# Sachin-A/TraceWeaver

Measured on AMD Instinct MI355X. Metric: spans/sec reconstructed + assignment accuracy vs ground truth, higher is better.
Workload: dtype int64 timestamps, f64 scores; 1 GPU; media_microservices shape (6 services, E in {1,1,1,1,2,4}), 100000 requests/service x 16 replicas per GPU, concurrency 1.6, two-pass reconstruction, device mixture refit; spans_per_gpu=25600000, spans_total=25600000, parallelism=units sharded, 1 rank(s), backend none

## Files before the change

### traceweaver_amd/csrc/tw_device.h

```cpp
#pragma once
#include <hip/hip_runtime.h>
#include <stdint.h>

#include "traceweaver_amd.h"

namespace tw {

constexpr int kMaxEp = TW_MAX_EP;
constexpr int kTopK = TW_TOPK;
constexpr int kMaxComp = TW_MAX_COMP;
constexpr int kMaxWin = TW_MAX_WINDOW;
constexpr int kCandWords = TW_CAND_WORDS;
constexpr int kEnumStretches = 8;
constexpr int kTile = 128;
constexpr int kCoop = 256;
constexpr int32_t kNoOwner = 0x7f7f7f7f;

struct UnitDev {
    int64_t in_off;
    int64_t ie_off;
    int64_t ep_off[kMaxEp + 1];
    int32_t n_in;
    int32_t E;
    int32_t nblk;
// ... 60 lines not shown
    int32_t* tkr_n;
    int32_t *tk_idx, *tkr_idx;
    double *tk_score, *tkr_score;
    int32_t* c_lo;
    int32_t* c_hi;
    uint64_t* c_bits;
    uint64_t* gone;
    uint8_t* gone_valid;
    int64_t* leaves_r;
    unsigned long long* frontier_big;
    int32_t* frontier_big_busy;
    int32_t frontier_big_slots;
    int32_t* frontier_busy;
    unsigned long long* frontier;
    int32_t* round_changed;
    int32_t* parent;
    int32_t* owner;
    double* gaps;
    const int64_t* gs_off;
    int64_t* unit_stats;
    int32_t* heavy_count;
    int32_t* heavy_next;
    int32_t *heavy_unit, *heavy_win;
    int32_t *tiny_unit, *tiny_win;
    int32_t *rheavy_unit, *rheavy_win, *rtiny_unit, *rtiny_win;
    int32_t *hard_unit, *hard_win;
    int32_t* heavy_in_count;
    int32_t* heavy_in_next;
    int32_t heavy_in_off[kMaxEp + 2];
    int32_t* enum_snap;
    int32_t* enum_stretch_next;
    int32_t *heavy_in_unit, *heavy_in_idx;
    int32_t* heavy_big_count;
    int32_t *heavy_big_unit, *heavy_big_idx;
    int32_t heavy_big_off[kMaxEp + 2];
    int32_t* heavy_big_part;
    int32_t* heavy_big_slot;
    int32_t part_off[kMaxEp + 2];
    int32_t split_twins;
    int32_t* part_used;
    int32_t defer_min_e;
    int32_t defer_cap;
    unsigned long long* defer_list;
    int32_t* defer_used;
    int32_t* defer_count;
    int32_t *part_lo, *part_hi;
    int32_t* part_lvl;
    int32_t* any_wide;
    int32_t* redo_count;
    int32_t* defer_refused;
    int32_t lean_min_e;
    int32_t tile_max_deep;
    int32_t lean_grid;
    double* pair_pool;
    int32_t* pair_busy;
    int32_t* fb_count;
    int32_t* fb_total;
    int32_t *fb_unit, *fb_idx, *fb_part, *fb_slot;
    int32_t* split_count;
    int32_t *split_unit, *split_idx, *split_slot, *split_parts;
    int32_t* part_n;
    int64_t* part_leaves;
    double* part_score;
    int32_t* part_idx;
    unsigned long long* part_bits;
    int32_t* part_logn;
    double* part_log_sc;
    unsigned long long* part_log_ix;
    int32_t* err;
    unsigned long long* prof;
};

__device__ __forceinline__ int32_t hi_word(double x) { return (int32_t)(__double_as_longlong(x) >> 32); }
__device__ __forceinline__ uint32_t lo_word(double x) { return (uint32_t)__double_as_longlong(x); }
__device__ __forceinline__ double with_hi(double x, int32_t hi) {
    return __longlong_as_double((long long)(((uint64_t)(uint32_t)hi << 32) | (uint64_t)lo_word(x)));
}
__device__ __forceinline__ double dnan() { return __longlong_as_double(0x7ff8000000000000LL); }
__device__ __forceinline__ double dinf() { return __longlong_as_double(0x7ff0000000000000LL); }

__device__ inline double tw_log(double x) {
    const double ln2_hi = 6.93147180369123816490e-01, ln2_lo = 1.90821492927058770002e-10,
                 two54 = 1.80143985094819840000e+16, Lg1 = 6.666666666666735130e-01,
                 Lg2 = 3.999999999940941908e-01, Lg3 = 2.857142874366239149e-01,
                 Lg4 = 2.222219843214978396e-01, Lg5 = 1.818357216161805012e-01,
                 Lg6 = 1.531383769920937332e-01, Lg7 = 1.479819860511658591e-01;
    int32_t k = 0, hx = hi_word(x);
    if (hx < 0x00100000) {
        if (((hx & 0x7fffffff) | lo_word(x)) == 0) return -dinf();
        if (hx < 0) return dnan();
        k -= 54;
        x *= two54;
        hx = hi_word(x);
    }
    if (hx >= 0x7ff00000) return x + x;
    k += (hx >> 20) - 1023;
    hx &= 0x000fffff;
    int32_t i = (hx + 0x95f64) & 0x100000;
    x = with_hi(x, hx | (i ^ 0x3ff00000));
    k += (i >> 20);
    double f = x - 1.0, dk = (double)k;
    if ((0x000fffff & (2 + hx)) < 3) {
        if (f == 0.0) return k == 0 ? 0.0 : dk * ln2_hi + dk * ln2_lo;
        double R = f * f * (0.5 - 0.33333333333333333 * f);
        return k == 0 ? f - R : dk * ln2_hi - ((R - dk * ln2_lo) - f);
    }
// ... 169 lines not shown
```

### traceweaver_amd/csrc/tw_engine.hip

```cpp
#include <algorithm>
#include <chrono>
#include <cmath>
#include <cstdio>
#include <cstdlib>
#include <cstring>
#include <functional>
#include <string>
#include <type_traits>
#include <vector>

#include <hip/hip_runtime.h>
#include <rocprim/rocprim.hpp>

#include "traceweaver_amd.h"
#include "tw_kernels.h"
#include "tw_fit.h"
#include "tw_eval.h"
#include "tw_skip.h"
#include "tw_load.h"
#include "tw_baselines.h"
#include "tw_stitch.h"
#include "tw_attr.h"
#include "tw_conf.h"
#include "tw_dist.h"
// ... 25 lines not shown
    uint32_t next() {
        if (idx >= 624) {
            for (int i = 0; i < 624; i++) {
                const uint32_t y = (mt[i] & 0x80000000u) | (mt[(i + 1) % 624] & 0x7fffffffu);
                mt[i] = mt[(i + 397) % 624] ^ (y >> 1) ^ ((y & 1u) ? 0x9908b0dfu : 0u);
            }
            idx = 0;
        }
        uint32_t y = mt[idx++];
        y ^= y >> 11;
        y ^= (y << 7) & 0x9d2c5680u;
        y ^= (y << 15) & 0xefc60000u;
        y ^= y >> 18;
        return y;
    }
    double random_sample() {
        const uint32_t a = next() >> 5, b = next() >> 6;
        return ((double)a * 67108864.0 + (double)b) / 9007199254740992.0;
    }
};

}

struct tw_engine {
    int device = 0;
    hipStream_t stream = nullptr;
    hipStream_t cls_stream[kMaxEp + 1] = {};
    hipEvent_t cls_ev[kMaxEp + 2] = {};
    hipStream_t sel_stream[3] = {};
    hipStream_t sel_stream2[3] = {};
    int64_t select_fork_min = 0;
    hipEvent_t prep_ev = nullptr;
    hipEvent_t post_fork[kMaxEp + 1] = {}, post_join[kMaxEp + 1][3] = {}, post_done[kMaxEp + 1] = {};
    hipEvent_t tile_ev[kMaxEp + 1] = {};
    hipStream_t cls_stream2[kMaxEp + 1] = {};
    hipEvent_t stretch_ev[kMaxEp + 1][kEnumStretches] = {}, stretch_done[kMaxEp + 1] = {};
    int enum_stretches = 1, stretch_min_tiles = 2048;
    int heavy_grid = 4096, select_grid = 0;
    int debug_lists = 0;
    int32_t first_lists[3][kMaxEp + 1] = {};
    hipEvent_t gate_ev = nullptr;
    int tile_gate = 0;
    int stage_min_tiles = 1024;
    int32_t *rank_in = nullptr, *rank_out = nullptr;
    bool class_params = false;
    int prio_min_e = 0, prio_high = 0;
    bool prio_any = false;
    int pipeline = 1;
    std::string err;
    int state = ST_EMPTY;
    int tile = kTile;
    int tile_threads = 2;
    int tile_single = 1;
    int block_params = 1;
    int tile_single_threads = 1;
    int coop = kCoop;
    std::vector<UnitDev> units;
    std::vector<TileDev> tiles;
    std::vector<int64_t> gs_off_h;
    std::vector<void*> allocs;
    void* arena = nullptr;
    size_t arena_cap = 0;
    bool arena_open = false;
    std::vector<std::pair<std::function<void(void*)>, size_t>> arena_req;
    Dev P{};
    int64_t n_ie = 0, n_gp = 0, n_slots = 0, n_gaps = 0;
    PairVI* agg_pair = nullptr;
    int32_t *agg_i32 = nullptr, *agg_i32b = nullptr;
    uint32_t *seg_in = nullptr, *seg_out = nullptr;
    int n_seg_out = 0;
    void* sort_tmp = nullptr;
    size_t sort_tmp_bytes = 0;
    double* mix_p_dev = nullptr;
    int32_t* mix_n_dev = nullptr;
    double* mix_c_dev = nullptr;
    double* gaps_sorted = nullptr;
    double* fit_models = nullptr;
    double* fit_uval = nullptr;
    int32_t *fit_ustart = nullptr, *fit_row_n = nullptr, *fit_row_uniq = nullptr;
    double* fit_centres = nullptr;
    double *fit_tape = nullptr, *fit_tape100 = nullptr;
    int64_t* fit_tape_off = nullptr;
    int64_t fit_tape_cap = 0;
    bool fit_runs_pending = false;
    bool fit_prepared = false;
    int tile_sub_max = 8;
    int32_t hard_pass1[kMaxEp + 1] = {};
    int8_t wide_pass1[kMaxEp + 1] = {};
    int32_t split_pass1[kMaxEp + 1] = {};
    int lean_pool = 512;
    bool pass1_done = false;
    std::vector<int32_t> fit_max_n;
    bool fit_max_n_valid = false;
    Mt19937 fit_rng;
    uint32_t fit_seed = 0;
    int32_t* slot_unit = nullptr;
    int32_t* tile_ids = nullptr;
    int32_t* ctr = nullptr;
    int64_t ctr_round_ints = 0, ctr_pass_ints = 0;
    int32_t tile_cls_off[kMaxEp + 2] = {};
    BlockRef* blk_tab = nullptr;
    int32_t blk_cls_off[kMaxEp + 2] = {};
    uint32_t *seg_gap = nullptr, *seg_gap_end = nullptr, *seg_gap_dst = nullptr;
    unsigned long long *comp_a = nullptr, *comp_b = nullptr;
    int64_t comp_cap = 0, n_gap_scored = 0;
    int32_t *truth = nullptr, *in_trace = nullptr;
// ... 745 lines not shown
    const unsigned grid_in = (unsigned)std::min<int64_t>((n_in + 255) / 256, 8192), grid_out = (unsigned)std::min<int64_t>((n_out + 255) / 256, 8192);
    const unsigned block = flat_threads(e);
    int64_t* d_is = const_cast<int64_t*>(P.in_start); int64_t* d_ie = const_cast<int64_t*>(P.in_end);
    int64_t* d_os = const_cast<int64_t*>(P.out_start); int64_t* d_oe = const_cast<int64_t*>(P.out_end);
    for (int side = 0; side < 2; side++) {
        const int64_t n = side == 0 ? n_in : n_out;
        const int64_t* vs = (const int64_t*)(side == 0 ? L.x : L.y); const int64_t* ve = (const int64_t*)(side == 0 ? L.xe : L.ye);
        const int32_t* rank = side == 0 ? L.rank_in : L.rank_out; const int32_t* row = side == 0 ? L.row_in : L.row_out;
        const int nrows = side == 0 ? P.n_units : e->n_seg_out;
        unsigned bs = 0, be = 0;
        rc = differing_bits(e, vs, n, &bs); if (rc != TW_OK) return rc;
        rc = differing_bits(e, ve, n, &be); if (rc != TW_OK) return rc;
        hipLaunchKernelGGL(k_load_iota, dim3(side == 0 ? grid_in : grid_out), dim3(block), 0, e->stream, perm, n);
        rc = load_sort_pass(e, rank, n, 32u, ka, kb, &perm, &perm_alt); if (rc != TW_OK) return rc;
        rc = load_sort_pass(e, ve, n, be, ka, kb, &perm, &perm_alt); if (rc != TW_OK) return rc;
        rc = load_sort_pass(e, vs, n, bs, ka, kb, &perm, &perm_alt); if (rc != TW_OK) return rc;
        rc = load_sort_pass(e, row, n, std::max(1u, bit_length((unsigned long long)std::max(nrows - 1, 1))), ka, kb, &perm, &perm_alt); if (rc != TW_OK) return rc;
        hipLaunchKernelGGL(k_load_place, dim3(side == 0 ? grid_in : grid_out), dim3(block), 0, e->stream, (const uint32_t*)perm, n, vs, ve,
                           side == 0 ? d_is : d_os, side == 0 ? d_ie : d_oe, side == 0 ? pos_in : pos_out);
        hipLaunchKernelGGL(k_load_local, dim3(side == 0 ? grid_in : grid_out), dim3(block), 0, e->stream, perm, row, (const uint32_t*)(side == 0 ? e->seg_in : e->seg_out), n);
        HIPCHK(hipGetLastError());
        int32_t* host = side == 0 ? in_perm : out_perm;
        if (host != nullptr) HIPCHK(hipMemcpyAsync(host, perm, sizeof(uint32_t) * n, hipMemcpyDeviceToHost, e->stream));
        HIPCHK(hipStreamSynchronize(e->stream));
    }
    hipLaunchKernelGGL(k_load_retruth, dim3(P.n_tiles), dim3(e->tile), 0, e->stream, L, (const int32_t*)pos_in, (const int32_t*)pos_out, e->truth,
                       has_trace ? e->in_trace : nullptr);
    HIPCHK(hipGetLastError());
    for (int u = 0; u < P.n_units; u++) {
        UnitDev& U = e->units[(size_t)u];
        U.tscale = std::ldexp(1.0, -kmax_h[(size_t)u]);
        U.float_time = 1;
        if (unit_time_scale != nullptr) unit_time_scale[u] = U.tscale;
    }
    HIPCHK(hipMemcpyAsync(const_cast<UnitDev*>(P.units), e->units.data(), sizeof(UnitDev) * e->units.size(), hipMemcpyHostToDevice, e->stream));
    HIPCHK(hipStreamSynchronize(e->stream));
    e->state = ST_LOADED; e->pass1_done = false;
    drop_batch_order(e);
    for (int E = 0; E <= kMaxEp; E++) { e->wide_pass1[E] = -1; e->hard_pass1[E] = -1; e->split_pass1[E] = -1; }
    return TW_OK;
}

extern "C" {

int tw_create(int device_id, tw_engine** out) {
    if (out == nullptr) return TW_ERR_ARG;
    *out = nullptr;
    tw_engine* e = new tw_engine();
    e->device = device_id;
    e->tile = std::min(std::max(env_int("TW_TILE", kTile), 1), kTile);
    e->tile_threads = std::min(std::max(env_int("TW_TILE_THREADS", 2), 1), 4);
    e->tile_single = env_int("TW_TILE_SINGLE", 1);
    e->block_params = env_int("TW_BLOCK_PARAMS", 1);
    e->tile_single_threads = std::min(std::max(env_int("TW_TILE_SINGLE_THREADS", 1), 1), 4);
    e->coop = std::min(std::max(env_int("TW_COOP_THREADS", kCoop), 1), kCoop);
    if (env_int("TW_SET_HW_QUEUES", 0) != 0) setenv("GPU_MAX_HW_QUEUES", "12", 0);
    hipError_t s = hipSetDevice(device_id);
    if (s == hipSuccess) s = hipStreamCreate(&e->stream);
    for (int i = 0; i < EV_COUNT && s == hipSuccess; i++) s = hipEventCreate(&e->ev[i]);
    for (int i = 0; i < SE_COUNT && s == hipSuccess; i++) s = hipEventCreate(&e->stage_ev[i]);
    const int prio_min_e = env_int("TW_PRIO_MIN_E", 0);
    int prio_least = 0, prio_greatest = 0;
    if (s == hipSuccess) s = hipDeviceGetStreamPriorityRange(&prio_least, &prio_greatest);
    e->prio_min_e = prio_min_e; e->prio_high = prio_greatest; e->prio_any = prio_greatest != prio_least;
    for (int i = 0; i <= kMaxEp + 1 && s == hipSuccess; i++) s = hipEventCreateWithFlags(&e->cls_ev[i], hipEventDisableTiming);
    if (s == hipSuccess) s = hipEventCreateWithFlags(&e->prep_ev, hipEventDisableTiming);
    for (int i = 0; i <= kMaxEp && s == hipSuccess; i++) {
        s = hipEventCreateWithFlags(&e->post_fork[i], hipEventDisableTiming);
        if (s == hipSuccess) s = hipEventCreateWithFlags(&e->tile_ev[i], hipEventDisableTiming);
        if (s == hipSuccess) s = hipEventCreateWithFlags(&e->post_done[i], hipEventDisableTiming);
        if (s == hipSuccess) s = hipEventCreateWithFlags(&e->stretch_done[i], hipEventDisableTiming);
        for (int j = 0; j < kEnumStretches && s == hipSuccess; j++) s = hipEventCreateWithFlags(&e->stretch_ev[i][j], hipEventDisableTiming);
        for (int j = 0; j < 3 && s == hipSuccess; j++) s = hipEventCreateWithFlags(&e->post_join[i][j], hipEventDisableTiming);
    }
    e->pipeline = env_int("TW_CLASS_PIPELINE", 1);
    e->sig_hash_bits = std::min(std::max(env_int("TW_SIG_HASH_BITS", 64), 1), 64);
    e->tile_gate = env_int("TW_TILE_GATE", 0);
    e->enum_stretches = std::min(std::max(env_int("TW_ENUM_STRETCHES", 1), 1), kEnumStretches);
    e->heavy_grid = std::max(env_int("TW_HEAVY_GRID", 4096), 64);
    e->select_grid = std::max(env_int("TW_SELECT_GRID", 0), 0);
    e->debug_lists = env_int("TW_DEBUG_LISTS", 0);
    e->select_fork_min = (int64_t)env_int("TW_SELECT_FORK_MIN", 0);
    e->stretch_min_tiles = std::max(env_int("TW_STRETCH_MIN_TILES", 2048), 1);
    e->stage_min_tiles = env_int("TW_STAGE_MIN_TILES", 1024);
    e->tile_sub_max = std::max(env_int("TW_TILE_SUB", 8), 1);
    e->lean_pool = std::min(std::max(env_int("TW_LEAN_POOL", 512), 1), 4096);
    if (s != hipSuccess) {
        fprintf(stderr, "tw_create: %s\n", hipGetErrorString(s));
        delete e;
        return TW_ERR_DEVICE;
    }
    *out = e;
    return TW_OK;
}

void tw_destroy(tw_engine* e) {
    if (e == nullptr) return;
    (void)hipSetDevice(e->device);
    free_all(e);
    order_unstage(e);
    if (e->arena != nullptr) (void)hipFree(e->arena);
    for (int i = 0; i < EV_COUNT; i++)
        if (e->ev[i]) (void)hipEventDestroy(e->ev[i]);
    for (int i = 0; i <= kMaxEp + 1; i++)
        if (e->cls_ev[i]) (void)hipEventDestroy(e->cls_ev[i]);
    for (int i = 1; i <= kMaxEp; i++)
// ... 149 lines not shown
        for (int cls = 1; cls <= kMaxEp; cls++) if (e->tile_cls_off[cls + 1] > e->tile_cls_off[cls]) deepest = cls;
        for (int cls = 1; cls < deepest; cls++) want |= e->select_fork_min > 0 && heavy_off_h[cls + 1] - heavy_off_h[cls] >= e->select_fork_min;
        for (int j = 0; j < 3 && want; j++)
            if (e->sel_stream2[j] == nullptr) HIPCHK(hipStreamCreate(&e->sel_stream2[j]));
    }
    const int64_t n_in_total = b->unit_in_off[b->n_units], n_out_total = b->ep_off[epi];
    if (n_in_total >= (1ll << 31) || n_out_total >= (1ll << 31)) return fail(e, TW_ERR_ARG, "batch exceeds 2^31 spans");
    if (gaps >= (1ll << 31)) return fail(e, TW_ERR_ARG, "batch too large: sum of nslot*n_in must stay below 2^31");
    std::vector<int32_t> slot_unit_h;
    std::vector<uint8_t> slot_scored_h;
    std::vector<uint32_t> seg_gap_h, seg_gap_end_h;
    for (int u = 0; u < b->n_units; u++) {
        const UnitDev& U = e->units[(size_t)u];
        const int E = U.E;
        for (int q = 0; q < U.nslot; q++) {
            bool scored;
            if (q < E) scored = U.npred[q] == 0;
            else if (q < E + E * E) {
                const int p = (q - E) / E, en = (q - E) % E;
                scored = false;
                for (int j = 0; j < U.npred[en]; j++) scored |= (U.pred_list[en][j] == p && U.pred_prim[en][j]);
            } else scored = true;
            slot_unit_h.push_back(u);
            slot_scored_h.push_back(scored ? 1 : 0);
            if (scored) {
                seg_gap_h.push_back((uint32_t)(e->gs_off_h[(size_t)u] + (int64_t)q * U.n_in));
                seg_gap_end_h.push_back((uint32_t)(e->gs_off_h[(size_t)u] + (int64_t)(q + 1) * U.n_in));
            }
        }
    }
    e->n_gap_rows = (int64_t)seg_gap_h.size();
    std::vector<uint32_t> seg_gap_dst_h(seg_gap_h.size());
    e->n_gap_scored = 0;
    for (size_t r = 0; r < seg_gap_h.size(); r++) { seg_gap_dst_h[r] = (uint32_t)e->n_gap_scored; e->n_gap_scored += seg_gap_end_h[r] - seg_gap_h[r]; }
    seg_in[(size_t)b->n_units] = (uint32_t)n_in_total;
    seg_out.push_back((uint32_t)n_out_total);
    e->n_seg_out = (int)seg_out.size() - 1;
    e->n_ie = ie; e->n_gp = gp; e->n_slots = slots; e->n_gaps = gaps;

    Dev& P = e->P;
    P = Dev{};
    P.n_units = b->n_units;
    P.n_tiles = (int32_t)e->tiles.size();
    P.tile_spans = e->tile;
    P.n_in_total = n_in_total;
    P.n_out_total = n_out_total;
    P.batch_size = b->batch_size;
    P.batch_mis = b->batch_size_mis;
    P.split_twins = env_int("TW_SPLIT_TWINS", 2);
    P.defer_min_e = env_int("TW_DEFER_MIN_E", 5);
    P.lean_min_e = env_int("TW_LEAN_MIN_E", 5);
    P.lean_grid = std::max(env_int("TW_LEAN_GRID", TW_LEAN_GRID), 1);
    P.tile_max_deep = std::min(std::max(env_int("TW_TILE_MAX_DEEP", kTileMax), 0), kTileMax);
    int rc;
    e->arena_req.clear();
    e->arena_open = true;
    UnitDev* d_units; TileDev* d_tiles; int64_t *d_is, *d_ie, *d_os, *d_oe, *d_gs;
    DEV_ALLOC(d_units, P.n_units); DEV_ALLOC(d_tiles, P.n_tiles);
    DEV_ALLOC(d_is, n_in_total); DEV_ALLOC(d_ie, n_in_total); DEV_ALLOC(d_os, n_out_total); DEV_ALLOC(d_oe, n_out_total);
    DEV_ALLOC(d_gs, P.n_units);
    DEV_ALLOC(P.in_end_sorted, n_in_total); DEV_ALLOC(P.out_end_sorted, n_out_total);
    DEV_ALLOC(P.gparam, gp * 4);
    DEV_ALLOC(e->mix_n_dev, slots); DEV_ALLOC(e->mix_p_dev, slots * kMaxComp * 3); DEV_ALLOC(e->mix_c_dev, slots * kMaxComp * 4);
    DEV_ALLOC(P.pm_val, n_in_total); DEV_ALLOC(P.pm_idx, n_in_total); DEV_ALLOC(P.pc, n_in_total + 1); DEV_ALLOC(P.seg, n_in_total);
    DEV_ALLOC(P.win_end, n_in_total); DEV_ALLOC(P.wid, n_in_total); DEV_ALLOC(P.w_last, n_in_total);
    DEV_ALLOC(P.unit_nwin, P.n_units); DEV_ALLOC(P.w_dirty, n_in_total); DEV_ALLOC(P.w_conf, n_in_total);
    DEV_ALLOC(P.tk_n, n_in_total); DEV_ALLOC(P.leaves, n_in_total); DEV_ALLOC(P.leaves0, n_in_total); DEV_ALLOC(P.chosen, n_in_total); DEV_ALLOC(P.rep, n_in_total);
    DEV_ALLOC(P.tkr_n, n_in_total);
    DEV_ALLOC(P.tk_idx, ie * kTopK); DEV_ALLOC(P.tkr_idx, ie * kTopK);
    DEV_ALLOC(P.tk_score, n_in_total * kTopK); DEV_ALLOC(P.tkr_score, n_in_total * kTopK);
    DEV_ALLOC(P.c_lo, ie); DEV_ALLOC(P.c_hi, ie); DEV_ALLOC(P.c_bits, ie * kCandWords); DEV_ALLOC(P.parent, ie);
    DEV_ALLOC(P.gone, ie * kCandWords); DEV_ALLOC(P.gone_valid, n_in_total); DEV_ALLOC(P.leaves_r, n_in_total);
    DEV_ALLOC(P.frontier, (int64_t)kFrontierSlots * 2 * kFrontierCap); 
    P.frontier_big_slots = (int32_t)std::min<int64_t>(std::max<int64_t>(n_in_total / 16384, kFrontierBigSlots), std::max(kFrontierBigSlots, 512));
    DEV_ALLOC(P.frontier_big, (int64_t)P.frontier_big_slots * 2 * kFrontierBigCap);
    DEV_ALLOC(P.pair_pool, (int64_t)kPairSlots * kPairSpill);
    DEV_ALLOC(P.owner, n_out_total);
    DEV_ALLOC(P.gaps, gaps);
    DEV_ALLOC(e->tile_ids, (int64_t)tile_ids_h.size());
    DEV_ALLOC(e->blk_tab, (int64_t)blk_tab_h.size());
    DEV_ALLOC(P.heavy_in_unit, n_in_total); DEV_ALLOC(P.heavy_in_idx, n_in_total);
    {
        int64_t big_total = 0, slots = 0, want = 0;
        for (int cls = 0; cls <= kMaxEp; cls++) want += 2 * part_extra(cls, heavy_off_h[cls + 1] - heavy_off_h[cls]);
        static const int64_t slots_max = (int64_t)std::max(env_int("TW_PART_SLOTS_MAX", 16 << 20), 1024);
        for (int cls = 0; cls <= kMaxEp; cls++) {
            const int64_t n_cls = heavy_off_h[cls + 1] - heavy_off_h[cls];
            int64_t extra = part_extra(cls, n_cls);
            if (want > slots_max && extra > 64) extra = std::max<int64_t>((int64_t)((double)extra * (double)slots_max / (double)want), std::min<int64_t>(n_cls / 8 + 64, extra));
            P.heavy_big_off[cls] = (int32_t)big_total; P.part_off[cls] = (int32_t)slots;
            big_total += n_cls + extra; slots += 2 * extra;
        }
        P.heavy_big_off[kMaxEp + 1] = (int32_t)big_total; P.part_off[kMaxEp + 1] = (int32_t)slots;
        DEV_ALLOC(P.heavy_big_unit, big_total); DEV_ALLOC(P.heavy_big_idx, big_total);
        DEV_ALLOC(P.heavy_big_part, big_total); DEV_ALLOC(P.heavy_big_slot, big_total);
        DEV_ALLOC(P.fb_unit, big_total); DEV_ALLOC(P.fb_idx, big_total); DEV_ALLOC(P.fb_part, big_total); DEV_ALLOC(P.fb_slot, big_total);
        DEV_ALLOC(P.split_unit, slots); DEV_ALLOC(P.split_idx, slots); DEV_ALLOC(P.split_slot, slots); DEV_ALLOC(P.split_parts, slots);
        DEV_ALLOC(P.part_n, slots); DEV_ALLOC(P.part_leaves, slots); DEV_ALLOC(P.part_score, slots * kTopK); DEV_ALLOC(P.part_idx, slots * kTopK * kMaxEp);
        DEV_ALLOC(P.part_bits, slots * kMaxEp * kCandWords);
        DEV_ALLOC(P.part_logn, slots); DEV_ALLOC(P.part_log_sc, slots * kPartLogCap); DEV_ALLOC(P.part_log_ix, slots * kPartLogCap);
        DEV_ALLOC(P.part_lo, slots); DEV_ALLOC(P.part_hi, slots); DEV_ALLOC(P.part_lvl, slots);
        int64_t deep = 0;
        for (int cls = std::max(P.defer_min_e, 3); cls <= kMaxEp; cls++) deep += heavy_off_h[cls + 1] - heavy_off_h[cls];
        P.defer_cap = (int32_t)(deep > 0 ? std::min<int64_t>(std::max<int64_t>(deep * kDeferListPerSpan, kDeferListMin), 1ll << 28) : 1);
        DEV_ALLOC(P.defer_list, P.defer_cap);
    }
// ... 1782 lines not shown
```

### traceweaver_amd/csrc/tw_tile.h

```cpp
#pragma once

namespace tw {

#ifndef TW_TILE_MAX
#define TW_TILE_MAX 256
#endif
constexpr int kTileMax = TW_TILE_MAX;
#ifndef TW_TILE_REPLAY_MAX
#define TW_TILE_REPLAY_MAX 256
#endif
constexpr int kTileReplayMax = TW_TILE_REPLAY_MAX;
__device__ __forceinline__ int pos_base(unsigned long long pk, int e) {
    int acc = 0;
    for (int f = 0; f < e; f++) acc += (int)((pk >> (8 * f)) & 255ull);
    return acc;
}
#ifndef TW_TILE_ITEMS
#define TW_TILE_ITEMS 768
#define TW_TILE_GRID 1024
#endif
constexpr int kSubTileSpans = kTile / 8;
template <int E, int SPANS = kTile>
struct TileCfg {
#ifdef TW_TILE_SMALL
    static constexpr int kSlice = 24, kItems = kMaxEp * 32, kGrid = kTileMax > 64 ? kTileMax : 64;
#else
    static constexpr int kSlice = SPANS < kTile ? 64 : (E <= 4 ? 192 : 160);
    static constexpr int kItems = SPANS < kTile ? kMaxEp * 32 : TW_TILE_ITEMS;
    static constexpr int kGrid = SPANS < kTile ? (kTileMax > 512 ? kTileMax : 512) : TW_TILE_GRID;
#endif
    static_assert(kItems >= kMaxEp * 32 && kGrid >= ((kTileMax + 3) & ~3) && kGrid % 4 == 0, "a single span must fit a segment");
};

__device__ __forceinline__ uint32_t div_small(uint32_t rest, uint32_t c) {
#ifdef TW_HOST_EMULATION
    const float rc = 1.0f / (float)c;
#else
    const float rc = __builtin_amdgcn_rcpf((float)c);
#endif
    return (uint32_t)(((float)rest + 0.5f) * rc);
}

__device__ __forceinline__ int fresh(int v) {
#ifndef TW_HOST_EMULATION
    asm volatile("" : "+v"(v));
#endif
    return v;
}

__device__ __forceinline__ double score_term_gap(const Scorer& S, int slot, long long gap) {
    const double x = (double)gap;
    if (S.pass == 1) {
        const double* g = S.gp + slot * 4;
        return term_gauss(g[0], g[3], g[2], x);
    }
    return score_term_mix_x(S, slot, x);
}

#ifdef TW_PROFILE_TILE
#ifndef TW_PROFILE_TILE_E
#define TW_PROFILE_TILE_E 4
#endif
#define TW_TILE_T0() long long _tp = wall_clock64(); const long long _tb = _tp; long long _ta[7] = {0, 0, 0, 0, 0, 0, 0}
#define TW_TILE_TICK(k) do { const long long _n = wall_clock64(); _ta[k] += _n - _tp; _tp = _n; } while (0)
#define TW_TILE_COUNT(k, v) do { if (E == TW_PROFILE_TILE_E && threadIdx.x == 0) atomicAdd((unsigned long long*)&P.prof[k], (unsigned long long)(v)); } while (0)
#define TW_TILE_FLUSH() do { if (E == TW_PROFILE_TILE_E && threadIdx.x == 0) { for (int _k = 0; _k < 7; _k++) atomicAdd((unsigned long long*)&P.prof[_k], (unsigned long long)_ta[_k]); \
    atomicAdd((unsigned long long*)&P.prof[7], (unsigned long long)(wall_clock64() - _tb)); atomicAdd((unsigned long long*)&P.prof[8], 1ull); } } while (0)
#else
#define TW_TILE_T0() do {} while (0)
#define TW_TILE_TICK(k) do {} while (0)
#define TW_TILE_COUNT(k, v) do {} while (0)
#define TW_TILE_FLUSH() do {} while (0)
#endif

#ifdef TW_HOST_EMULATION
#define TW_TILE_ATTR
#else
#define TW_TILE_ATTR __attribute__((amdgpu_waves_per_eu(SINGLE ? 8 : (E <= 4 ? 4 : 2))))
#endif
template <int E, int SPANS = kTile, bool SINGLE = false>
__global__ void __launch_bounds__(4 * kTile) TW_TILE_ATTR k_enumerate_tile(Dev P, int pass, const int32_t* tile_ids, int n_tiles_e, int sub_tiles) {
    static_assert(!SINGLE || E == 1, "the lean path is the one of a single endpoint");
    if (*P.err != 0) return;
    typedef TileCfg<E, SPANS> C;
    constexpr int SL = C::kSlice;
    const int vb = xcd_tile(blockIdx.x, n_tiles_e * sub_tiles);
    const int tile = tile_ids[vb / sub_tiles];
    const TileDev T = P.tiles[tile];
    const UnitDev& U = P.units[T.unit];
    const int t = threadIdx.x, nt = blockDim.x;
    const int sub_spans = P.tile_spans / sub_tiles, first = T.first + (vb % sub_tiles) * sub_spans;
    const int ns = min(sub_spans, min(P.tile_spans, U.n_in - T.first) - (vb % sub_tiles) * sub_spans);
    if (ns <= 0) return;
    __shared__ int32_t s_is[SPANS], s_ie[SPANS];
    __shared__ int32_t sl_st[E][SL], sl_en[E][SL];
    __shared__ int32_t s_A[E], s_B[E];
    __shared__ uint16_t s_lo[E][SPANS];
    __shared__ uint32_t s_cm[E][SPANS];
    __shared__ uint32_t s_bits[E][SPANS];
    __shared__ int32_t s_item0[SPANS + 1], s_grid0[SPANS + 1], s_leaves[SPANS];
    __shared__ uint8_t s_amb[SPANS];
    __shared__ unsigned long long s_cn[SPANS];
    __shared__ int32_t s_wtot[4 * kTile / 64][2];
    __shared__ double t_root[C::kItems], t_close[C::kItems];
    __shared__ uint16_t it_idx[C::kItems];
    __shared__ double g_sc[C::kGrid];
    __shared__ uint8_t g_span[C::kGrid], g_rank[C::kGrid];
    __shared__ int32_t s_segend, s_anyamb;
    const bool live = t < ns;
    const int i = first + (live ? t : 0);
    const int64_t base = P.in_start[U.in_off + first];
    const int64_t in_start = P.in_start[U.in_off + i], in_end = P.in_end[U.in_off + i];
    const int64_t* os[E];
    const int64_t* oe[E];
#pragma unroll
    for (int e = 0; e < E; e++) { os[e] = P.out_start + U.ep_off[e]; oe[e] = P.out_end + U.ep_off[e]; }
    for (int x = t; x < E; x += nt) { s_A[x] = 0x7fffffff; s_B[x] = 0; }
    uint32_t dag_pm[E], dag_np[E], dag_pl[E];
    uint32_t ordered = 0;
#pragma unroll
    for (int e = 0; e < E; e++) {
        dag_pm[e] = U.pred_mask[e];
        dag_np[e] = U.npred[e];
        uint32_t pk = 0;
#pragma unroll
        for (int j = 0; j < E; j++) pk |= (j < (int)dag_np[e] ? ((uint32_t)U.pred_list[e][j] | ((uint32_t)U.pred_prim[e][j] << 3)) : 0u) << (4 * j);
        dag_pl[e] = pk;
        ordered |= dag_pm[e];
    }
    TW_TILE_T0();
    int32_t lo[E], hi[E];
    if (pass == 1) {
#pragma unroll
        for (int e = E - 1; e >= 0; e--) {
            const int n = (int)(U.ep_off[e + 1] - U.ep_off[e]);
            int64_t tmax = in_end;
#pragma unroll
            for (int f = e + 1; f < E; f++) {
                if (!((U.succ_mask[e] >> f) & 1)) continue;
                const int nf = (int)(U.ep_off[f + 1] - U.ep_off[f]);
                const int anchor = hi[f] >= 0 ? hi[f] : nf - 1;
                const int64_t st = os[f][anchor];
                if (st < tmax) tmax = st;
            }
            if (U.skip) {
                lo[e] = lower_bound_i64(os[e], n, in_start);
                hi[e] = upper_bound_i64(os[e], n, tmax) - 1;
            } else {
                lo[e] = bound_near<false>(os[e], n, in_start, i);
                hi[e] = bound_near<true>(os[e], n, tmax, lo[e]) - 1;
            }
        }
        if (live) {
#pragma unroll
            for (int e = 0; e < E; e++) { P.c_lo[ie_index(U, e, i)] = lo[e]; P.c_hi[ie_index(U, e, i)] = hi[e]; }
        }
    } else {
#pragma unroll
        for (int e = 0; e < E; e++) { lo[e] = P.c_lo[ie_index(U, e, i)]; hi[e] = P.c_hi[ie_index(U, e, i)]; }
    }
// ... 227 lines not shown
                if (s_amb[s]) continue;
                const int r = it_rank[k], si = first + s;
                P.tk_score[tks_index(U, r, si)] = s_sc[k];
                P.tk_idx[tk_index(U, r, 0, si)] = s_A[0] + (int)it_idx[k];
            }
            const int tl = fresh(t);
            const bool replay = s_anyamb != 0 && here && s_mine[tl] && s_amb[tl] && (tl + 1) * (kTopK + 1) <= C::kItems && nitem1 <= kTileReplayMax;
            auto start_of = [&](int, int pos) -> int32_t { return sl_st[0][it_idx[ks + pos]]; };
            RegHeap RH;
            RH.clear(E);
            if (replay) {
                for (int pos = 0; pos < nitem1; pos++) {
                    const double sc = s_sc[ks + pos];
                    if (!(sc == sc) || RH.below_root(sc)) continue;
                    RH.push(sc, (unsigned long long)pos, start_of);
                }
            }
            if (s_anyamb != 0) group_sync();
            if (replay) {
                double* hs = s_sc + tl * (kTopK + 1);
                uint8_t* hx = it_rank + tl * (kTopK + 1);
#pragma unroll
                for (int k = 0; k < kTopK; k++) { hs[k] = RH.s[k]; hx[k] = (uint8_t)RH.x[k]; }
                py_sort_desc(hs, hx, RH.n, [&](double sa, unsigned long long xa, double sb, unsigned long long xb) { return RH.lt(sa, xa, sb, xb, start_of); });
                const int si = first + tl;
                for (int k = 0; k < RH.n; k++) {
                    P.tk_score[tks_index(U, k, si)] = hs[k];
                    P.tk_idx[tk_index(U, k, 0, si)] = s_A[0] + (int)it_idx[ks + (int)hx[k]];
                }
                s_amb[tl] = 0;
            }
            if (here && s_mine[tl] && !s_amb[tl]) {
                const int i1 = first + tl;
                const int64_t g = U.in_off + i1;
                P.tk_n[g] = nitem1 < kTopK ? nitem1 : kTopK;
                P.leaves[g] = nitem1;
                if (pass == 1) P.leaves0[g] = nitem1;
                P.rep[g] = 0;
                if (pass == 1) {
                    P.c_bits[ie_index(U, 0, i1) * kCandWords] = (uint64_t)s_cm[0][tl];
                    for (int w = 1; w < kCandWords; w++) P.c_bits[ie_index(U, 0, i1) * kCandWords + w] = (uint64_t)(uint32_t)fresh(0);
                }
            }
            group_sync();
            TW_TILE_TICK(6);
            seg = send;
        }
        TW_TILE_FLUSH();
        const int te = fresh(t);
        heavy_append<E>(P, live && s_mine[te] != 0 && s_amb[te] != 0, true, false, T.unit, first + (live ? te : 0), 0, 0, false, te & 63);
        return;
    } else
    for (int seg = 0; seg < ns;) {
        if (t == 0) { s_segend = ns; s_anyamb = 0; }
        group_sync();
        if (live && t >= seg && (s_item0[t + 1] - s_item0[seg] > C::kItems || s_grid0[t + 1] - s_grid0[seg] > C::kGrid)) atomicMin(&s_segend, t);
        group_sync();
        const int send = s_segend;
        const int it0 = s_item0[seg], nIt = s_item0[send] - it0, g0 = s_grid0[seg], nG = s_grid0[send] - g0;
        TW_TILE_TICK(2);
        TW_TILE_COUNT(9, 1); TW_TILE_COUNT(10, nIt); TW_TILE_COUNT(11, nG);
        for (int k = t; k < nIt; k += nt) {
            const int s = span_of(s_item0, seg, send, it0 + k);
            int j = it0 + k - s_item0[s], es = 0;
            uint32_t m = 0;
            bool found = false;
#pragma unroll
            for (int e = 0; e < E; e++)
                if (!found) { m = s_cm[e][s]; const int c = __popcll((unsigned long long)m); if (j < c) { es = e; found = true; } else j -= c; }
            const int idx = (int)s_lo[es][s] + nth_set_bit((unsigned long long)m, j);
            int32_t st = 0, en = 0;
            bool is_root = false;
#pragma unroll
            for (int e = 0; e < E; e++) if (e == es) { st = sl_st[e][idx]; en = sl_en[e][idx]; is_root = dag_np[e] == 0; }
            S.gp = P.gparam + (U.gp_off + (int64_t)((first + s) / P.batch_size) * U.nslot) * 4;
            t_root[k] = is_root ? score_term_gap(S, slot_root(E, es), (long long)st - s_is[s]) : 0.0;
            t_close[k] = score_term_gap(S, slot_close(E, es), (long long)s_ie[s] - en);
            it_idx[k] = (uint16_t)idx;
        }
        group_sync();
        TW_TILE_TICK(3);
        for (int g = t; g < nG; g += nt) {
            const int s = span_of(s_grid0, seg, send, g0 + g);
            int32_t kx[E], ix[E], st[E], en[E];
            const int gi = g0 + g - s_grid0[s];
            uint32_t real = 1;
            {
                const unsigned long long pk = s_cn[s];
#pragma unroll
                for (int e = 0; e < E; e++) real *= (uint32_t)((pk >> (8 * e)) & 255ull);
            }
            bool ok = (uint32_t)gi < real;
            decode(s, ok ? gi : 0, it0, kx, ix);
#pragma unroll
            for (int e = 0; e < E; e++) {
                st[e] = sl_st[e][ix[e]]; en[e] = sl_en[e][ix[e]];
#pragma unroll
                for (int p = 0; p < e; p++)
                    if (((dag_pm[e] >> p) & 1) && en[p] > st[e]) ok = false;
            }
            double sj = 0.0;
            if (ok) {
                int last = 0;
                int32_t last_end = en[0];
#pragma unroll
                for (int e = 1; e < E; e++) if (en[e] > last_end) { last_end = en[e]; last = e; }
                S.gp = P.gparam + (U.gp_off + (int64_t)((first + s) / P.batch_size) * U.nslot) * 4;
#pragma unroll
                for (int e = 0; e < E; e++) {
                    const int np = (int)dag_np[e];
#pragma unroll
                    for (int j = 0; j < E; j++) {
                        if (j >= np) continue;
                        const uint32_t pj = (dag_pl[e] >> (4 * j)) & 15u;
                        if (!(pj & 8u)) continue;
                        const int p = (int)(pj & 7u);
                        int32_t pend = 0;
#pragma unroll
                        for (int q = 0; q < E; q++) if (q == p) pend = en[q];
                        sj += score_term_gap(S, slot_prim(E, p, e), (long long)st[e] - pend);
                    }
                    if (np == 0) sj += t_root[kx[e]];
                    if (e == last) sj += t_close[kx[e]];
                }
                if (ordered) {
                    atomicAdd(&s_leaves[s], 1);
                    if (pass == 1) {
#pragma unroll
                        for (int e = 0; e < E; e++) atomicOr(&s_bits[e][s], 1u << (ix[e] - (int)s_lo[e][s]));
                    }
                }
            }
            g_sc[g] = ok ? sj : dnan();
            g_span[g] = (uint8_t)s;
        }
        group_sync();
        TW_TILE_TICK(4);
        for (int g = t; g < nG; g += nt) {
            const double my = g_sc[g];
            int rank = kTopK;
            if (my == my) {
                const int s = g_span[g];
                const int gs = s_grid0[s] - g0, ge = s_grid0[s + 1] - g0;
                rank = 0;
                bool partner = false;
                int eq = 0;
                for (int h0 = gs; h0 < ge && rank < kTopK; h0 += 4) {
                    const double o0 = g_sc[h0], o1 = g_sc[h0 + 1], o2 = g_sc[h0 + 2], o3 = g_sc[h0 + 3];
                    rank += (o0 > my) + (o1 > my) + (o2 > my) + (o3 > my);
                    eq += (o0 == my) + (o1 == my) + (o2 == my) + (o3 == my);
                }
                if (eq > 1 && rank < kTopK) {
                    int32_t ka[E], ia[E];
                    decode(s, g - gs, it0, ka, ia);
                    for (int h = gs; h < ge; h++) {
                        if (h == g || !(g_sc[h] == my)) continue;
                        int32_t kb[E], ib[E];
                        decode(s, h - gs, it0, kb, ib);
                        int ord = 0;
                        bool done = false;
#pragma unroll
                        for (int e = 0; e < E; e++)
                            if (!done && ia[e] != ib[e]) {
                                const int32_t a = sl_st[e][ia[e]], b = sl_st[e][ib[e]];
                                ord = b > a ? 1 : (b < a ? -1 : 0);
                                done = true;
                            }
                        if (ord > 0) rank++;
                        else if (ord == 0) partner = true;
                    }
                }
                if (partner && rank < kTopK) { s_amb[s] = 1; s_anyamb = 1; }
            }
            g_rank[g] = (uint8_t)(rank < kTopK ? rank : kTopK);
        }
        group_sync();
        TW_TILE_TICK(5);
        for (int g = t; g < nG; g += nt) {
            if (g_rank[g] >= kTopK) continue;
            const int s = g_span[g];
            if (s_amb[s]) continue;
            int32_t kx[E], ix[E];
            decode(s, g0 + g - s_grid0[s], it0, kx, ix);
            const int k = g_rank[g], si = first + s;
            P.tk_score[tks_index(U, k, si)] = g_sc[g];
#pragma unroll
            for (int e = 0; e < E; e++) P.tk_idx[tk_index(U, k, e, si)] = s_A[e] + ix[e];
        }
        if (s_anyamb != 0) group_sync();
        if (s_anyamb != 0 && live && t >= seg && t < send && mine && s_amb[t] && (t + 1) * (kTopK + 1) <= C::kItems && s_leaves[t] <= kTileReplayMax) {
            RegHeap RH;
            RH.clear(E);
            const unsigned long long pk = s_cn[t];
            auto start_of = [&](int e, int pos) -> int32_t { return sl_st[e][it_idx[s_item0[t] - it0 + pos_base(pk, e) + pos]]; };
            uint32_t real = 1;
#pragma unroll
            for (int e = 0; e < E; e++) real *= (uint32_t)((pk >> (8 * e)) & 255ull);
            const int gs = s_grid0[t] - g0;
            for (uint32_t gi = 0; gi < real; gi++) {
                const double sc = g_sc[gs + gi];
                if (!(sc == sc) || RH.below_root(sc)) continue;
                unsigned long long x = 0;
                uint32_t rest = gi;
#pragma unroll
                for (int e = E - 1; e >= 0; e--) {
                    const uint32_t c = (uint32_t)((pk >> (8 * e)) & 255ull);
                    const uint32_t q = c == 1 ? rest : div_small(rest, c);
                    x |= (unsigned long long)(rest - q * c) << (8 * e);
                    rest = q;
                }
                RH.push(sc, x, start_of);
            }
            double* hs = t_root + t * (kTopK + 1);
            unsigned long long* hx = reinterpret_cast<unsigned long long*>(t_close + t * (kTopK + 1));
#pragma unroll
            for (int k = 0; k < kTopK; k++) { hs[k] = RH.s[k]; hx[k] = RH.x[k]; }
            py_sort_desc(hs, hx, RH.n, [&](double sa, unsigned long long xa, double sb, unsigned long long xb) { return RH.lt(sa, xa, sb, xb, start_of); });
            const int si = first + t;
            for (int k = 0; k < RH.n; k++) {
                P.tk_score[tks_index(U, k, si)] = hs[k];
#pragma unroll
                for (int e = 0; e < E; e++)
                    P.tk_idx[tk_index(U, k, e, si)] = s_A[e] + (int)it_idx[s_item0[t] - it0 + pos_base(pk, e) + (int)((hx[k] >> (8 * e)) & 255ull)];
            }
            s_amb[t] = 0;
        }
        if (live && t >= seg && t < send && mine && !s_amb[t]) {
// ... 24 lines not shown
```

Baseline: 1.335 billion spans/s.

## Prune top-K ranking for long spans via bucket maxima and survivor compaction

```diff
diff --git a/traceweaver_amd/csrc/tw_device.h b/traceweaver_amd/csrc/tw_device.h
--- a/traceweaver_amd/csrc/tw_device.h
+++ b/traceweaver_amd/csrc/tw_device.h
@@ -136,6 +136,7 @@
     int32_t lean_min_e;
     int32_t tile_max_deep;
     int32_t lean_grid;
+    int32_t tile_rank;
     double* pair_pool;
     int32_t* pair_busy;
     int32_t* fb_count;
diff --git a/traceweaver_amd/csrc/tw_engine.hip b/traceweaver_amd/csrc/tw_engine.hip
--- a/traceweaver_amd/csrc/tw_engine.hip
+++ b/traceweaver_amd/csrc/tw_engine.hip
@@ -101,6 +101,7 @@
     int tile = kTile;
     int tile_threads = 2;
     int tile_single = 1;
+    int tile_rank = 1;
     int block_params = 1;
     int tile_single_threads = 1;
     int coop = kCoop;
@@ -952,6 +953,7 @@
     e->tile_threads = std::min(std::max(env_int("TW_TILE_THREADS", 2), 1), 4);
     e->tile_single = env_int("TW_TILE_SINGLE", 1);
     e->block_params = env_int("TW_BLOCK_PARAMS", 1);
+    e->tile_rank = env_int("TW_TILE_RANK", 1) != 0 ? 1 : 0;
     e->tile_single_threads = std::min(std::max(env_int("TW_TILE_SINGLE_THREADS", 1), 1), 4);
     e->coop = std::min(std::max(env_int("TW_COOP_THREADS", kCoop), 1), kCoop);
     if (env_int("TW_SET_HW_QUEUES", 0) != 0) setenv("GPU_MAX_HW_QUEUES", "12", 0);
@@ -1207,6 +1209,7 @@
     P.lean_min_e = env_int("TW_LEAN_MIN_E", 5);
     P.lean_grid = std::max(env_int("TW_LEAN_GRID", TW_LEAN_GRID), 1);
     P.tile_max_deep = std::min(std::max(env_int("TW_TILE_MAX_DEEP", kTileMax), 0), kTileMax);
+    P.tile_rank = e->tile_rank;
     int rc;
     e->arena_req.clear();
     e->arena_open = true;
diff --git a/traceweaver_amd/csrc/tw_tile.h b/traceweaver_amd/csrc/tw_tile.h
--- a/traceweaver_amd/csrc/tw_tile.h
+++ b/traceweaver_amd/csrc/tw_tile.h
@@ -10,6 +10,17 @@
 #define TW_TILE_REPLAY_MAX 256
 #endif
 constexpr int kTileReplayMax = TW_TILE_REPLAY_MAX;
+#ifndef TW_TILE_RANK_DIRECT
+#define TW_TILE_RANK_DIRECT 32
+#endif
+constexpr int kRankDirect = TW_TILE_RANK_DIRECT;
+constexpr int kRankMinLong = (kRankDirect & ~3) + 4;
+constexpr int kRankBuckets = 5;
+static_assert(kRankDirect >= 24, "the maxima and counters of a segment's long spans lie in one byte per tuple slot");
+__device__ __forceinline__ uint32_t score_key32(double v) {
+    const unsigned long long u = (unsigned long long)__double_as_longlong(v + 0.0);
+    return (uint32_t)(((u >> 63) ? ~u : (u | (1ull << 63))) >> 32);
+}
 __device__ __forceinline__ int pos_base(unsigned long long pk, int e) {
     int acc = 0;
     for (int f = 0; f < e; f++) acc += (int)((pk >> (8 * f)) & 255ull);
@@ -105,7 +116,8 @@
     __shared__ double t_root[C::kItems], t_close[C::kItems];
     __shared__ uint16_t it_idx[C::kItems];
     __shared__ double g_sc[C::kGrid];
-    __shared__ uint8_t g_span[C::kGrid], g_rank[C::kGrid];
+    __shared__ uint8_t g_span[C::kGrid];
+    __shared__ uint32_t g_aux[C::kGrid / 4];
     __shared__ int32_t s_segend, s_anyamb;
     const bool live = t < ns;
     const int i = first + (live ? t : 0);
@@ -439,6 +451,16 @@
         return;
     } else
     for (int seg = 0; seg < ns;) {
+        constexpr int kLong = (C::kGrid - kRankMinLong) / kRankMinLong + 1;
+        constexpr bool kRankFits = kLong * (kRankBuckets + 1) + 1 <= C::kGrid / 4 && C::kGrid * 4 <= C::kItems * 8 && C::kGrid <= 65536;
+        static_assert(kRankBuckets == kTopK && C::kGrid <= C::kItems * 8, "a subset of slots per entry of the list; a rank per slot in t_root");
+        uint32_t* const r_max = g_aux;
+        int32_t* const r_cnt = reinterpret_cast<int32_t*>(g_aux + kLong * kRankBuckets);
+        uint8_t* const g_rank = reinterpret_cast<uint8_t*>(t_root);
+        uint16_t* const r_sub = reinterpret_cast<uint16_t*>(t_close);
+        uint16_t* const r_all = r_sub + C::kGrid;
+        const bool compact = kRankFits && P.tile_rank != 0;
+        if (compact) for (int x = fresh(t); x < kLong * (kRankBuckets + 1) + 1; x += nt) g_aux[x] = 0u;
         if (t == 0) { s_segend = ns; s_anyamb = 0; }
         group_sync();
         if (live && t >= seg && (s_item0[t + 1] - s_item0[seg] > C::kItems || s_grid0[t + 1] - s_grid0[seg] > C::kGrid)) atomicMin(&s_segend, t);
@@ -520,15 +542,70 @@
             }
             g_sc[g] = ok ? sj : dnan();
             g_span[g] = (uint8_t)s;
+            if (compact && ok && s_grid0[s + 1] - s_grid0[s] > kRankDirect) {
+                uint32_t* b = r_max + ((g - gi) / kRankMinLong) * kRankBuckets + gi % kRankBuckets;
+                const uint32_t key = score_key32(sj);
+                if (key > *(volatile uint32_t*)b) atomicMax(b, key);
+            }
         }
         group_sync();
         TW_TILE_TICK(4);
+        auto order_equal = [&](int s, const int32_t (&ia)[E], int hrel) -> int {
+            int32_t kb[E], ib[E];
+            decode(s, hrel, it0, kb, ib);
+            int ord = 0;
+            bool done = false;
+#pragma unroll
+            for (int e = 0; e < E; e++)
+                if (!done && ia[e] != ib[e]) {
+                    const int32_t a = sl_st[e][ia[e]], b = sl_st[e][ib[e]];
+                    ord = b > a ? 1 : (b < a ? -1 : 0);
+                    done = true;
+                }
+            return ord;
+        };
+        if (compact) {
+            const int tr = fresh(t);
+            for (int gb = 0; gb < nG; gb += nt) {
+                const int g = gb + tr, lane = tr & 63;
+                bool surv = false;
+                int sub0 = 0;
+                if (g < nG) {
+                    const double my = g_sc[g];
+                    const int s = g_span[g];
+                    const int gs = s_grid0[s] - g0, ge = s_grid0[s + 1] - g0;
+                    if (ge - gs > kRankDirect && my == my) {
+                        const uint32_t* b = r_max + (gs / kRankMinLong) * kRankBuckets;
+                        uint32_t lk = b[0];
+#pragma unroll
+                        for (int j = 1; j < kRankBuckets; j++) lk = b[j] < lk ? b[j] : lk;
+                        surv = score_key32(my) >= lk;
+                        sub0 = gs;
+                    }
+                }
+                const int at = wave_append(&r_cnt[kLong], surv, lane);
+                if (surv) r_all[at] = (uint16_t)g;
+                unsigned long long todo = __ballot(surv);
+                while (todo != 0ull) {
+                    const int leader = __ffsll((long long)todo) - 1;
+                    const int lead0 = __shfl(sub0, leader);
+                    const bool with = surv && sub0 == lead0;
+                    const unsigned long long m = __ballot(with);
+                    int base = 0;
+                    if (lane == leader) base = atomicAdd(&r_cnt[lead0 / kRankMinLong], __popcll(m));
+                    base = __shfl(base, leader);
+                    if (with) r_sub[lead0 + base + __popcll(m & ((1ull << lane) - 1ull))] = (uint16_t)g;
+                    todo &= ~m;
+                }
+            }
+        }
         for (int g = t; g < nG; g += nt) {
             const double my = g_sc[g];
             int rank = kTopK;
+            const int s = g_span[g];
+            const int gs = s_grid0[s] - g0, ge = s_grid0[s + 1] - g0;
+            if (compact && ge - gs > kRankDirect) { g_rank[g] = (uint8_t)kTopK; continue; }
             if (my == my) {
-                const int s = g_span[g];
-                const int gs = s_grid0[s] - g0, ge = s_grid0[s + 1] - g0;
                 rank = 0;
                 bool partner = false;
                 int eq = 0;
@@ -542,17 +619,7 @@
                     decode(s, g - gs, it0, ka, ia);
                     for (int h = gs; h < ge; h++) {
                         if (h == g || !(g_sc[h] == my)) continue;
-                        int32_t kb[E], ib[E];
-                        decode(s, h - gs, it0, kb, ib);
-                        int ord = 0;
-                        bool done = false;
-#pragma unroll
-                        for (int e = 0; e < E; e++)
-                            if (!done && ia[e] != ib[e]) {
-                                const int32_t a = sl_st[e][ia[e]], b = sl_st[e][ib[e]];
-                                ord = b > a ? 1 : (b < a ? -1 : 0);
-                                done = true;
-                            }
+                        const int ord = order_equal(s, ia, h - gs);
                         if (ord > 0) rank++;
                         else if (ord == 0) partner = true;
                     }
@@ -560,6 +627,38 @@
                 if (partner && rank < kTopK) { s_amb[s] = 1; s_anyamb = 1; }
             }
             g_rank[g] = (uint8_t)(rank < kTopK ? rank : kTopK);
+        }
+        if (compact) {
+            group_sync();
+            const int nsv = r_cnt[kLong];
+            for (int k = fresh(t); k < nsv; k += nt) {
+                const int g = r_all[k];
+                const double my = g_sc[g];
+                const int s = g_span[g];
+                const int gs = s_grid0[s] - g0;
+                const int n = r_cnt[gs / kRankMinLong];
+                const uint16_t* sub = r_sub + gs;
+                int rank = 0, eq = 0;
+                for (int h = 0; h < n && rank < kTopK; h++) {
+                    const double o = g_sc[sub[h]];
+                    rank += (o > my);
+                    eq += (o == my);
+                }
+                bool partner = false;
+                if (eq > 1 && rank < kTopK) {
+                    int32_t ka[E], ia[E];
+                    decode(s, g - gs, it0, ka, ia);
+                    for (int h = 0; h < n; h++) {
+                        const int hg = sub[h];
+                        if (hg == g || !(g_sc[hg] == my)) continue;
+                        const int ord = order_equal(s, ia, hg - gs);
+                        if (ord > 0) rank++;
+                        else if (ord == 0) partner = true;
+                    }
+                }
+                if (partner && rank < kTopK) { s_amb[s] = 1; s_anyamb = 1; }
+                g_rank[g] = (uint8_t)(rank < kTopK ? rank : kTopK);
+            }
         }
         group_sync();
         TW_TILE_TICK(5);
```

Measured after the change: 1.367 billion spans/s (median of 6 runs). 2.4% higher.
